# pixray/pixray

Hardware: AMD Instinct MI355X
Metric: optimisation iters/sec, VQGAN 256^2 + ViT-B/32 + 64 cutouts (higher is better)
Workload: dtype fp16

## Files before the change

### include/prx.h

```cpp
#ifndef PRX_H_
#define PRX_H_
#include <stddef.h>
#include <stdint.h>

#ifdef __cplusplus
extern "C" {
#endif

#define PRX_ABI_VERSION 3

typedef void* prx_stream_t;

const char* prx_last_error(void);
int prx_abi_version(void);
int prx_device_info(int* cu_count, char* arch_name, int arch_name_len);


#define PRX_ACT_NONE 0
#define PRX_ACT_QUICKGELU 1
#define PRX_ACT_MUL_DQUICKGELU 2
#define PRX_ACT_RELU 3
#define PRX_ACT_MUL_RELUMASK 4
#define PRX_ACT_RELUMASK_POST 5
#define PRX_ACT_GELU 6
// ... 106 lines not shown
int prx_k_image_head_bwd_im2col(const float* x, int ldc, const float* gimg, void* col, int ldk, int C, int H, int W, int h16,
                                const float* gscale, prx_stream_t s);
int prx_k_grad_scale(const float* g, size_t n, float* part, int nparts, int target_log2, float* scale2, prx_stream_t s);
int prx_k_grad_scale_multi(const float* const* gs, const size_t* ns, int count, float* part, int nparts_each, int target_log2,
                           float* scale2, prx_stream_t s);
int prx_k_scale_dev(float* x, size_t n, const float* scale, void* out16, int h16, prx_stream_t s);
int prx_k_f32_to_op16(const float* in, void* out16, size_t n, int h16, prx_stream_t s);
int prx_k_add_f32(const float* a, const float* b, float* out, size_t n, prx_stream_t s);

int prx_k_rn_pack_conv3x3(const float* w, void* Wf, void* Wd, int Cout, int Cin, int prec, prx_stream_t s);
int prx_k_stem1_fwd(const float* cut, const float* mm, const float* w, const float* b, void* out, int N, int S, int CO, int prec,
                    prx_stream_t s);
int prx_k_stem1_bwd(const void* g, const float* w, float* dY, int N, int S, int CO, const float* oscale_dev, int prec, prx_stream_t s);
int prx_k_avgpool2_fwd(const void* x, void* out, int N, int H, int W, int C, int prec, prx_stream_t s);
int prx_k_avgpool2_bwd(const float* g, const void* mask, float* dx_f32, void* dx_op, int N, int H, int W, int C, int prec,
                       prx_stream_t s);
int prx_k_relu_mask(float* g, const void* out, void* g_op, size_t n, int prec, prx_stream_t s);
int prx_k_tokens_fwd(const float* x, const float* pos, void* t, int N, int P, int C, int prec, prx_stream_t s);
int prx_k_tokens_bwd(const float* dt, float* dx, int N, int P, int C, int prec, prx_stream_t s);
int prx_k_tok0_gather(const void* t, void* out, int N, int T, int C, int prec, prx_stream_t s);
int prx_k_tok0_scatter(const void* g0, void* dt, int N, int T, int C, int prec, prx_stream_t s);
int prx_k_cnx_pack_dw(const float* w, void* pack, int C, int prec, prx_stream_t s);
int prx_k_cnx_dwconv(const void* x, const void* pack, const float* bias, const float* add, void* out_op, float* out_f32, int N, int H,
                     int W, int C, int flip, int prec, prx_stream_t s);
int prx_k_cnx_space_to_depth(const void* in, void* out, int N, int H, int W, int C, int prec, prx_stream_t s);
int prx_k_cnx_depth_to_space(const void* in, void* out, int N, int H, int W, int C, int prec, prx_stream_t s);
int prx_k_cnx_avgpool_fwd(const void* x, float* out, int N, int HW, int C, int prec, prx_stream_t s);
int prx_k_cnx_avgpool_bwd(const float* g, float* dx_f32, void* dx_op, int N, int HW, int C, int prec, prx_stream_t s);
int prx_k_cnx_layernorm_fwd(const void* x, int x_f32, const float* gamma, const float* beta, void* out_op, float* out_f32, float* mean,
                            float* rstd, int rows, int C, float eps, int group, int prec, prx_stream_t s);
int prx_k_cnx_layernorm_bwd(const float* g, const void* x, int x_f32, const float* gamma, const float* mean, const float* rstd,
                            void* dx_op, float* dx_f32, int rows, int C, int group, int prec, prx_stream_t s);
int prx_k_minmax(const float* x, size_t n, float* part, int nparts, float* mm, prx_stream_t s);
int prx_k_patchify_fwd(const float* cut, const float* mm, void* A, int prec, int N, int S, int P, int T, float m0, float m1, float m2,
                       float s0, float s1, float s2, prx_stream_t s);
int prx_k_patchify_bwd_reduce(const float* cut, const float* mm, const float* dA, double* acc, int N, int S, int P, int T, float m0,
                              float m1, float m2, float s0, float s1, float s2, prx_stream_t s);
int prx_k_patchify_bwd_apply(const float* cut, const float* mm, const float* dA, const double* acc, float* gcut, int N, int S, int P,
                             int T, float m0, float m1, float m2, float s0, float s1, float s2, prx_stream_t s);
int prx_k_preproc_bwd_reduce(const float* cut, const float* mm, const float* dY, double* acc, int N, int S, prx_stream_t s);
int prx_k_preproc_bwd_apply(const float* cut, const float* mm, const float* dY, const double* acc, float* gcut, int N, int S,
                            prx_stream_t s);
int prx_k_pool_fwd(const float* img, float* pooled, int* argmax, const unsigned char* mask, int C, int H, int W, int S, prx_stream_t s);
int prx_k_pool_bwd(const float* g, const int* argmax, const unsigned char* mask, float* gimg, int C, int H, int W, int S, prx_stream_t s);
int prx_k_rescale_fwd(const float* pooled, float* base, int C, int S, int Hb, int Wb, prx_stream_t s);
int prx_k_rescale_bwd(const float* g_base, float* g_pooled, int C, int S, int Hb, int Wb, prx_stream_t s);
int prx_k_warp_a_fwd(const float* src, int Hs, int Ws, const double* desc, float* out, int n_cut, int Ha, int Wa, prx_stream_t s);
int prx_k_warp_a_bwd(const float* g, int Hs, int Ws, const double* desc, float* uv, float* gsrc_priv, float* gsrc, int n_cut, int Ha,
                     int Wa, int form, prx_stream_t s);
int prx_k_warp_b_fwd(const float* a, int Ha, int Wa, const double* desc, const float* noise, float* out, int n_cut, int S,
                     prx_stream_t s);
int prx_k_warp_b_bwd(const float* a, int Ha, int Wa, const double* desc, const float* g, float* grgb, float* uv, float* ga, int n_cut,
                     int S, float* maps_scratch, size_t maps_scratch_bytes, int form, prx_stream_t s);
int prx_k_vgg_pack(const float* w, void* Wf, void* Wd, int Cout, int Cin, int CiP, int prec, prx_stream_t s);
int prx_k_vgg_input(const float* x, void* out, int HW, int prec, prx_stream_t s);
int prx_k_vgg_input_grad(const float* d, float* gx, int HW, const float* unscale, prx_stream_t s);
int prx_k_vgg_maxpool(const void* x, void* out, void* arg, int H, int W, int C, int prec, prx_stream_t s);
int prx_k_vgg_combine(const float* above, const void* arg, const float* gcap, const void* act, void* gpre, int H, int W, int C,
                      const float* gscale, int prec, prx_stream_t s);
int prx_k_pack_transpose_op(const float* in, void* out, int R, int C, int prec, prx_stream_t s);
int prx_k_vit_add_cls_pos(float* x, const float* cls, const float* pos, int N, int T, int W, prx_stream_t s);
int prx_k_vit_embed_tokens(const float* x, const float* cls, const float* pos, void* out, int out16, int N, int T, int W,
                           prx_stream_t s);
int prx_k_vit_gelu_f32(const float* t, float* io, size_t n, int bwd, prx_stream_t s);
int prx_k_vit_scale_f32(float* x, size_t n, float scale, int blocks, prx_stream_t s);
int prx_k_text_embed(const int* tokens, const float* emb, const float* pos, float* x, int* eot, int n, int ctx, int W, int vocab,
                     prx_stream_t s);
int prx_k_gather_rows(const float* x, const int* eot, float* out, int n, int ctx, int W, prx_stream_t s);
int prx_k_l2norm_fwd(const float* e, float* out, int n, int D, prx_stream_t s);
int prx_k_l2norm_bwd(const float* e, const float* g, float* de, int n, int D, prx_stream_t s);
int prx_k_vqgan_pack_conv3x3(const float* w, void* Wf, void* Wd, int Cout, int Cin, int CoP, int prec, prx_stream_t s);
int prx_k_vqgan_enc_pack_conv3x3(const float* w, void* Wf, int Cout, int Cin, int CiP, prx_stream_t s);
int prx_k_colminmax(const float* w, float* mn, float* mx, int rows, int D, prx_stream_t s);


typedef struct prx_vqgan prx_vqgan;
typedef struct prx_vqgan_config {
    int ch;
    int ch_mult[8];
    int n_mult;
    int num_res_blocks;
    int attn_resolution;
    int resolution;
    int z_channels;
    int embed_dim;
    int n_embed;
    int out_ch;
    int latent_h, latent_w;
    int precision;
} prx_vqgan_config;
int prx_vqgan_create(prx_vqgan** out, const prx_vqgan_config* cfg, const float* const* weights, int n_weights,
                     prx_stream_t s);
void prx_vqgan_destroy(prx_vqgan* h);
int prx_vqgan_z_bounds(prx_vqgan* h, float* zmin, float* zmax, prx_stream_t s);
int prx_vqgan_synth(prx_vqgan* h, const float* z, float* img, int* indices, int quantize, prx_stream_t s);
int prx_vqgan_synth_backward(prx_vqgan* h, const float* g_img, float* dz, prx_stream_t s);
long long prx_vqgan_debug_stage(prx_vqgan* h, int stage, float* dst, long long max_floats, prx_stream_t stream);

typedef struct prx_vqgan_enc prx_vqgan_enc;
int prx_vqgan_enc_create(prx_vqgan_enc** out, const prx_vqgan_config* cfg, int in_channels, int H, int W,
                         const float* const* weights, int n_weights, prx_stream_t s);
void prx_vqgan_enc_destroy(prx_vqgan_enc* h);
int prx_vqgan_encode(prx_vqgan_enc* h, const float* img, float* z, float* z_pre, int* indices, prx_stream_t s);

typedef struct prx_vgg16 prx_vgg16;
int prx_vgg16_create(prx_vgg16** out, const float* const* weights, int n_weights, int max_h, int max_w, int precision,
// ... 299 lines not shown
```

### pixray_amd/csrc/cutouts.hip

```cpp
#include "cutouts.h"
#include <algorithm>
#include <stdlib.h>
#include <stdio.h>

namespace {

constexpr int DESC_WORDS = 36;
enum { D_M1 = 0, D_M2 = 9, D_MODE1 = 18, D_MODE2 = 19, D_FILL = 20, D_JIT = 21, D_SAT = 22, D_HUE = 23,
       D_SATFIRST = 24, D_NOISE = 25, D_GRID1 = 26, D_GRID2 = 27,
       D_WOX = 28, D_WOY = 29, D_WW = 30, D_WH = 31,
       D_SEED = 32 };
enum { GRID_MESH = 0, GRID_AFFINE = 1, GRID_AFFINE_AC = 2, GRID_MESH_AC = 3 };
enum { MODE_IDENT = 0, MODE_ZEROS = 1, MODE_BORDER = 2, MODE_REFLECT = 3, MODE_FILL = 4,
       MODE_REFLECT_AC = 5 };

inline int ew_grid(size_t total) { return (int)std::min<size_t>((total + 255) / 256, 16384); }

__device__ __forceinline__ int win_start(int i, int in, int out) { return (int)(((long long)i * in) / out); }
__device__ __forceinline__ int win_end(int i, int in, int out) { return (int)((((long long)(i + 1)) * in + out - 1) / out); }

__global__ __launch_bounds__(256) void pool_fwd_kernel(const float* __restrict__ img, float* __restrict__ pooled,
                                                       int* __restrict__ argmax, const unsigned char* __restrict__ mask,
                                                       int C, int H, int W, int S) {
    const int total = C * S * S;
    for (int idx = blockIdx.x * blockDim.x + threadIdx.x; idx < total; idx += gridDim.x * blockDim.x) {
        const int x = idx % S, y = (idx / S) % S, c = idx / (S * S);
        const int y0 = win_start(y, H, S), y1 = win_end(y, H, S);
        const int x0 = win_start(x, W, S), x1 = win_end(x, W, S);
        float sum = 0.f, mx = -INFINITY;
        int am = y0 * W + x0;
        for (int yy = y0; yy < y1; ++yy)
            for (int xx = x0; xx < x1; ++xx) {
                float v = img[((size_t)c * H + yy) * W + xx];
                sum += v;
                if (v > mx || v != v) { mx = v; am = yy * W + xx; }
            }
        pooled[idx] = (mask && mask[idx]) ? 0.f : 0.5f * (sum / (float)((y1 - y0) * (x1 - x0)) + mx);
        argmax[idx] = am;
    }
}

__global__ __launch_bounds__(256) void pool_bwd_kernel(const float* __restrict__ g, const int* __restrict__ argmax,
                                                       const unsigned char* __restrict__ mask, float* __restrict__ gimg, int C, int H,
                                                       int W, int S) {
    const int total = C * H * W;
    for (int idx = blockIdx.x * blockDim.x + threadIdx.x; idx < total; idx += gridDim.x * blockDim.x) {
        const int xx = idx % W, yy = (idx / W) % H, c = idx / (H * W);
        int ya = (int)(((long long)yy * S) / H), xa = (int)(((long long)xx * S) / W);
        while (ya > 0 && win_end(ya - 1, H, S) > yy) --ya;
        while (xa > 0 && win_end(xa - 1, W, S) > xx) --xa;
        float acc = 0.f;
        for (int y = ya; y < S && win_start(y, H, S) <= yy; ++y) {
            const int y0 = win_start(y, H, S), y1 = win_end(y, H, S);
            if (yy >= y1) continue;
// ... 479 lines not shown
            }
        }
    if (COOP) {
#pragma unroll
        for (int c = 0; c < 3; ++c)
#pragma unroll
            for (int o = 32; o > 0; o >>= 1) acc[c] += __shfl_xor(acc[c], o, 64);
    }
    return total;
}

__device__ __forceinline__ void gather_tile(const GatherStage& st, const StageMap& sm, TileStage& ts, int tx0, int ty0, int sx, int sy,
                                            bool live, float (&out)[3]) {
    if (threadIdx.x == 0) {
        int x0, x1, y0, y1;
        ts.w = 0; ts.h = 0; ts.x0 = 0; ts.y0 = 0;
        const float ua = fmaxf((float)tx0 - 1.f, sm.ulo), ub = fminf((float)(tx0 + TILE_W) + 1.f, sm.uhi);
        const float va = fmaxf((float)ty0 - 1.f, sm.vlo), vb = fminf((float)(ty0 + TILE_W) + 1.f, sm.vhi);
        if (ub > ua && vb > va && preimage_box(sm, ua, ub, va, vb, st.Wd, st.Hd, x0, x1, y0, y1) &&
            (x1 - x0 + 1) * (y1 - y0 + 1) <= STAGE_CAP) {
            ts.x0 = x0; ts.y0 = y0; ts.w = x1 - x0 + 1; ts.h = y1 - y0 + 1;
        }
    }
    __syncthreads();
    {
        const int cnt = ts.w * ts.h;
        const size_t plane = (size_t)st.Hd * st.Wd;
        for (int k = threadIdx.x; k < cnt; k += 256) {
            const size_t o = (size_t)(ts.y0 + k / ts.w) * st.Wd + (ts.x0 + k % ts.w);
            ts.uv[k] = st.uv[o];
            ts.g[0][k] = st.g[o]; ts.g[1][k] = st.g[plane + o]; ts.g[2][k] = st.g[2 * plane + o];
        }
    }
    __syncthreads();
    float acc[3] = {0.f, 0.f, 0.f};
    int work = 0;
    if (live) work = gather_pixel<false>(st, sm, ts, sx, sy, acc, HEAVY);
    unsigned long long heavy = __ballot(live && work > HEAVY);
    while (heavy) {
        const int src = __ffsll((long long)heavy) - 1;
        heavy &= heavy - 1;
        const int hx = __shfl(sx, src, 64), hy = __shfl(sy, src, 64);
        float a2[3] = {0.f, 0.f, 0.f};
        gather_pixel<true>(st, sm, ts, hx, hy, a2, 0);
        if ((int)(threadIdx.x & 63) == src) { acc[0] = a2[0]; acc[1] = a2[1]; acc[2] = a2[2]; }
    }
    out[0] = acc[0]; out[1] = acc[1]; out[2] = acc[2];
}

struct TileRects {
    float ua[MAXR * MAXR], ub[MAXR * MAXR], va[MAXR * MAXR], vb[MAXR * MAXR];
    int x0[MAXR * MAXR], y0[MAXR * MAXR], bw[MAXR * MAXR], cnt[MAXR * MAXR];
};
struct TileScatter {
    int nrect;
    TileRects rect;
    float acc[4][3][TILE_W * TILE_W];
};
struct WaveScatter {
    TileRects rect;
    float acc[3][TILE_W * TILE_W];
};

__device__ __forceinline__ void scatter_candidate(const GatherStage& st, float* __restrict__ a0, float* __restrict__ a1, float* __restrict__ a2,
                                                  int tx0, int ty0, float ua, float ub, float va, float vb, float2 q, float g0, float g1, float g2) {
    if (!(q.x >= ua && q.x < ub && q.y >= va && q.y < vb)) return;
    const Taps t = make_taps(q.x, q.y, st.Ws, st.Hs, st.mode);
    const int lx = t.x0 - tx0, ly = t.y0 - ty0;
    const bool cx0 = t.vx0 && lx >= 0 && lx < TILE_W, cx1 = t.vx1 && lx + 1 >= 0 && lx + 1 < TILE_W;
    const bool cy0 = t.vy0 && ly >= 0 && ly < TILE_W, cy1 = t.vy1 && ly + 1 >= 0 && ly + 1 < TILE_W;
    if (!((cx0 || cx1) && (cy0 || cy1))) return;
    const float e = 1.f - t.wx, s_ = 1.f - t.wy;
    const float w00 = s_ * e, w01 = s_ * t.wx, w10 = t.wy * e, w11 = t.wy * t.wx;
    const int p00 = ly * TILE_W + lx;
    if (cx0 && cy0) { atomicAdd(&a0[p00], g0 * w00); atomicAdd(&a1[p00], g1 * w00); atomicAdd(&a2[p00], g2 * w00); }
    if (cx1 && cy0) { atomicAdd(&a0[p00 + 1], g0 * w01); atomicAdd(&a1[p00 + 1], g1 * w01); atomicAdd(&a2[p00 + 1], g2 * w01); }
    if (cx0 && cy1) { atomicAdd(&a0[p00 + TILE_W], g0 * w10); atomicAdd(&a1[p00 + TILE_W], g1 * w10); atomicAdd(&a2[p00 + TILE_W], g2 * w10); }
    if (cx1 && cy1) { atomicAdd(&a0[p00 + TILE_W + 1], g0 * w11); atomicAdd(&a1[p00 + TILE_W + 1], g1 * w11); atomicAdd(&a2[p00 + TILE_W + 1], g2 * w11); }
}

template <int STRIDE>
__device__ __forceinline__ void scatter_rect(const GatherStage& st, const TileRects& tr, int r, int tid, float* __restrict__ a0,
                                             float* __restrict__ a1, float* __restrict__ a2, int tx0, int ty0) {
    constexpr int U = 4;
    const size_t plane = (size_t)st.Hd * st.Wd;
    const float ua = tr.ua[r], ub = tr.ub[r], va = tr.va[r], vb = tr.vb[r];
    const int bx0 = tr.x0[r], by0 = tr.y0[r], bw = tr.bw[r], cnt = tr.cnt[r];
    const float ibw = 1.f / (float)bw;
    for (int k0 = tid; k0 < cnt; k0 += STRIDE * U) {
        float2 q[U]; float g0[U], g1[U], g2[U];
#pragma unroll
        for (int j = 0; j < U; ++j) {
            const int k = k0 + STRIDE * j;
            q[j] = make_float2(-INFINITY, -INFINITY);
            g0[j] = g1[j] = g2[j] = 0.f;
            if (k < cnt) {
                int ky = (int)((float)k * ibw);
                int kx = k - ky * bw;
                if (kx < 0) { --ky; kx += bw; } else if (kx >= bw) { ++ky; kx -= bw; }
                const size_t o = (size_t)(by0 + ky) * st.Wd + (bx0 + kx);
                q[j] = st.uv[o];
                g0[j] = st.g[o]; g1[j] = st.g[plane + o]; g2[j] = st.g[2 * plane + o];
            }
        }
#pragma unroll
        for (int j = 0; j < U; ++j) scatter_candidate(st, a0, a1, a2, tx0, ty0, ua, ub, va, vb, q[j], g0[j], g1[j], g2[j]);
    }
}

__device__ __forceinline__ void scatter_tile(const GatherStage& st, const StageMap& sm, TileScatter& ts, int tx0, int ty0, float (&out)[3]) {
    const int tid = threadIdx.x, wave = tid >> 6;
    if (tid == 0) {
        int n = 0;
        const int sx0 = max(tx0, 0), sx1 = min(tx0 + TILE_W - 1, st.Ws - 1);
        const int sy0 = max(ty0, 0), sy1 = min(ty0 + TILE_W - 1, st.Hs - 1);
        if (sx0 <= sx1 && sy0 <= sy1) {
            float xa[MAXR], xb[MAXR], ya[MAXR], yb[MAXR];
            const int nx = tile_intervals(st.mode, sx0, sx1, st.Ws, sm.ulo, sm.uhi, xa, xb);
            const int ny = tile_intervals(st.mode, sy0, sy1, st.Hs, sm.vlo, sm.vhi, ya, yb);
            for (int j = 0; j < ny; ++j)
                for (int i = 0; i < nx; ++i) {
                    int x0, x1, y0, y1;
                    if (!preimage_box(sm, xa[i], xb[i], ya[j], yb[j], st.Wd, st.Hd, x0, x1, y0, y1)) continue;
                    ts.rect.ua[n] = xa[i]; ts.rect.ub[n] = xb[i]; ts.rect.va[n] = ya[j]; ts.rect.vb[n] = yb[j];
                    ts.rect.x0[n] = x0; ts.rect.y0[n] = y0; ts.rect.bw[n] = x1 - x0 + 1; ts.rect.cnt[n] = (x1 - x0 + 1) * (y1 - y0 + 1);
                    ++n;
                }
        }
        ts.nrect = n;
    }
#pragma unroll
    for (int c = 0; c < 3; ++c)
#pragma unroll
        for (int w = 0; w < 4; ++w) ts.acc[w][c][tid] = 0.f;
    __syncthreads();
    const int nrect = ts.nrect;
    for (int r = 0; r < nrect; ++r) scatter_rect<256>(st, ts.rect, r, tid, ts.acc[wave][0], ts.acc[wave][1], ts.acc[wave][2], tx0, ty0);
    __syncthreads();
#pragma unroll
    for (int c = 0; c < 3; ++c) out[c] = ((ts.acc[0][c][tid] + ts.acc[1][c][tid]) + ts.acc[2][c][tid]) + ts.acc[3][c][tid];
}

__device__ __forceinline__ void scatter_tile_wave(const GatherStage& st, const StageMap& sm, WaveScatter& ts, int tx0, int ty0, float (&out)[4][3]) {
    const int lane = threadIdx.x & 63;
#pragma unroll
    for (int c = 0; c < 3; ++c)
#pragma unroll
        for (int j = 0; j < 4; ++j) ts.acc[c][lane + 64 * j] = 0.f;
    if (lane < MAXR * MAXR) {
        int cnt = 0;
        const int sx0 = max(tx0, 0), sx1 = min(tx0 + TILE_W - 1, st.Ws - 1);
        const int sy0 = max(ty0, 0), sy1 = min(ty0 + TILE_W - 1, st.Hs - 1);
        if (sx0 <= sx1 && sy0 <= sy1) {
            float xa[MAXR], xb[MAXR], ya[MAXR], yb[MAXR];
            const int nx = tile_intervals(st.mode, sx0, sx1, st.Ws, sm.ulo, sm.uhi, xa, xb);
            const int ny = tile_intervals(st.mode, sy0, sy1, st.Hs, sm.vlo, sm.vhi, ya, yb);
            const int i = lane % MAXR, j = lane / MAXR;
            if (i < nx && j < ny) {
                const float ua = i == 0 ? xa[0] : (i == 1 ? xa[1] : xa[2]), ub = i == 0 ? xb[0] : (i == 1 ? xb[1] : xb[2]);
                const float va = j == 0 ? ya[0] : (j == 1 ? ya[1] : ya[2]), vb = j == 0 ? yb[0] : (j == 1 ? yb[1] : yb[2]);
                int x0, x1, y0, y1;
                if (preimage_box(sm, ua, ub, va, vb, st.Wd, st.Hd, x0, x1, y0, y1)) {
                    ts.rect.ua[lane] = ua; ts.rect.ub[lane] = ub; ts.rect.va[lane] = va; ts.rect.vb[lane] = vb;
                    ts.rect.x0[lane] = x0; ts.rect.y0[lane] = y0; ts.rect.bw[lane] = x1 - x0 + 1;
                    cnt = (x1 - x0 + 1) * (y1 - y0 + 1);
                }
            }
        }
        ts.rect.cnt[lane] = cnt;
    }
    __builtin_amdgcn_s_waitcnt(0xc07f);
    __builtin_amdgcn_wave_barrier();
    for (int r = 0; r < MAXR * MAXR; ++r) {
        if (ts.rect.cnt[r] == 0) continue;
        scatter_rect<64>(st, ts.rect, r, lane, ts.acc[0], ts.acc[1], ts.acc[2], tx0, ty0);
    }
    __builtin_amdgcn_s_waitcnt(0xc07f);
    __builtin_amdgcn_wave_barrier();
#pragma unroll
    for (int j = 0; j < 4; ++j)
#pragma unroll
        for (int c = 0; c < 3; ++c) out[j][c] = ts.acc[c][lane + 64 * j];
}

__device__ __forceinline__ void write_stage_map(StageMap* __restrict__ maps, int n, const StageWords& w, int Wd, int Hd, int Ws, int Hs) {
    if (maps == nullptr || blockIdx.x != 0 || threadIdx.x != 0) return;
    StageMap sm{};
    if (w.mode != MODE_IDENT) build_stage_map(sm, w.m, w.gtype, Wd, Hd, Ws, Hs);
    maps[n] = sm;
}

__global__ __launch_bounds__(256) void uv_kernel(const double* __restrict__ desc, float2* __restrict__ uv, StageMap* __restrict__ maps,
                                                 int Wd, int Hd, int Ws, int Hs) {
// ... 107 lines not shown
    const StageWords w = stage_words(d, 2);
    const SrcWin q = src_window(d);
    write_stage_map(maps, n, w, S, S, q.ww, q.wh);
    const bool jit = d[D_JIT] != 0.0;
    if (w.mode == MODE_IDENT && !jit) return;
    const unsigned plane = (unsigned)S * (unsigned)S, stride = gridDim.x * blockDim.x;
    float2* uvn = uv + (size_t)n * plane;
    if (!jit) {
        for (unsigned pix = blockIdx.x * blockDim.x + threadIdx.x; pix < plane; pix += stride) {
            int x, y;
            pixel_xy(pix, (unsigned)S, x, y);
            float u, v;
            project(w.m, w.gtype, x, y, S, S, q.ww, q.wh, u, v);
            uvn[pix] = make_float2(u, v);
        }
        return;
    }
    const bool sat_first = d[D_SATFIRST] != 0.0;
    const float sat = (float)d[D_SAT], hue = (float)d[D_HUE];
    const size_t aplane = (size_t)Ha * Wa;
    const float* an = a + (size_t)n * 3 * aplane + (size_t)q.oy * Wa + q.ox;
    const float* gn = g + (size_t)n * 3 * plane;
    float* grn = grgb + (size_t)n * 3 * plane;
    for (unsigned pix = blockIdx.x * blockDim.x + threadIdx.x; pix < plane; pix += stride) {
        int x, y;
        pixel_xy(pix, (unsigned)S, x, y);
        Taps t = ident_taps(x, y);
        if (w.mode != MODE_IDENT) {
            float u, v;
            project(w.m, w.gtype, x, y, S, S, q.ww, q.wh, u, v);
            uvn[pix] = make_float2(u, v);
            t = make_taps(u, v, q.ww, q.wh, w.mode);
        }
        const float fillc = fill_term(t, w.fillv);
        Dual<3> rgb[3];
        float gin[3];
#pragma unroll
        for (int c = 0; c < 3; ++c) {
            rgb[c] = cst<3>(sample_plane(an + c * aplane, Wa, t) + fillc);
            rgb[c].d[c] = 1.f;
            gin[c] = gn[(size_t)c * plane + pix];
        }
        jitter_d<3>(rgb, sat, hue, sat_first);
#pragma unroll
        for (int i = 0; i < 3; ++i)
            grn[(size_t)i * plane + pix] = gin[0] * rgb[0].d[i] + gin[1] * rgb[1].d[i] + gin[2] * rgb[2].d[i];
    }
}

template <int FORM, int STAGE>
__global__ __launch_bounds__(FORM == 1 ? 64 : 256) void warp_bwd_kernel(const double* __restrict__ desc, const float* __restrict__ g,
                                                                        const float* __restrict__ grgb, const float2* __restrict__ uv,
                                                                        const StageMap* __restrict__ maps, float* __restrict__ out,
                                                                        int Wd, int Hd, int Wo, int Ho) {
    constexpr int NT = FORM == 1 ? 64 : 256;
    constexpr int PPT = TILE_W * TILE_W / NT;
    const int n = blockIdx.y;
    const double* d = desc + (size_t)n * DESC_WORDS;
    const int mode = (int)d[STAGE == 1 ? D_MODE1 : D_MODE2];
    const int ox = STAGE == 1 ? 0 : (int)d[D_WOX], oy = STAGE == 1 ? 0 : (int)d[D_WOY];
    const int ww = STAGE == 1 ? Wo : (int)d[D_WW], wh = STAGE == 1 ? Ho : (int)d[D_WH];
    const auto in_window = [&](int sx, int sy) { return STAGE == 1 || (sx >= 0 && sx < ww && sy >= 0 && sy < wh); };
    const size_t plane = (size_t)Hd * Wd, oplane = (size_t)Ho * Wo;
    const float* gi = (STAGE == 2 && d[D_JIT] != 0.0 ? grgb : g) + (size_t)n * 3 * plane;
    float* go = out + (size_t)n * 3 * oplane;
    const int tiles = (Wo + TILE_W - 1) / TILE_W;
    const int ax0 = (blockIdx.x % tiles) * TILE_W, ay0 = (blockIdx.x / tiles) * TILE_W;
    float o[PPT][3];
    if (mode == MODE_IDENT) {
#pragma unroll
        for (int j = 0; j < PPT; ++j) {
            const int p = threadIdx.x + NT * j, ax = ax0 + (p & 15), ay = ay0 + (p >> 4), sx = ax - ox, sy = ay - oy;
            const bool live = ax < Wo && ay < Ho && in_window(sx, sy) && sx < Wd && sy < Hd;
#pragma unroll
            for (int c = 0; c < 3; ++c) o[j][c] = live ? gi[(size_t)c * plane + (size_t)sy * Wd + sx] : 0.f;
        }
    } else {
        const GatherStage st{mode, Wd, Hd, ww, wh, gi, uv + (size_t)n * plane};
        const int tx0 = ax0 - ox, ty0 = ay0 - oy;
        if constexpr (FORM == 2) {
            __shared__ StageMap sm;
            __shared__ TileStage ts;
            if (threadIdx.x == 0) build_stage_map(sm, d + (STAGE == 1 ? D_M1 : D_M2), (int)d[STAGE == 1 ? D_GRID1 : D_GRID2], Wd, Hd, ww, wh);
            __syncthreads();
            const int ax = ax0 + (threadIdx.x & 15), ay = ay0 + (threadIdx.x >> 4), sx = ax - ox, sy = ay - oy;
            gather_tile(st, sm, ts, tx0, ty0, sx, sy, ax < Wo && ay < Ho && in_window(sx, sy), o[0]);
        } else if constexpr (FORM == 0) {
            __shared__ TileScatter ts;
            const StageMap sm = maps[n];
            scatter_tile(st, sm, ts, tx0, ty0, o[0]);
        } else {
            __shared__ WaveScatter ts;
            const StageMap sm = maps[n];
            scatter_tile_wave(st, sm, ts, tx0, ty0, o);
        }
    }
#pragma unroll
    for (int j = 0; j < PPT; ++j) {
        const int p = threadIdx.x + NT * j, ax = ax0 + (p & 15), ay = ay0 + (p >> 4);
        if (!(ax < Wo && ay < Ho)) continue;
        const bool live = in_window(ax - ox, ay - oy);
#pragma unroll
        for (int c = 0; c < 3; ++c) go[(size_t)c * oplane + (size_t)ay * Wo + ax] = live ? o[j][c] : 0.f;
    }
}

__device__ __forceinline__ void resize_taps(int o, int in, int outn, int& i0, int& i1, float& w1) {
    float src = ((float)o + 0.5f) * ((float)in / (float)outn) - 0.5f;
    if (src < 0.f) src = 0.f;
    i0 = (int)src;
    i1 = i0 + (i0 < in - 1 ? 1 : 0);
    w1 = src - (float)i0;
}
__global__ __launch_bounds__(256) void rescale_fwd_kernel(const float* __restrict__ p, float* __restrict__ out, int C, int S, int Hb, int Wb) {
    const size_t total = (size_t)C * Hb * Wb;
    for (size_t idx = (size_t)blockIdx.x * blockDim.x + threadIdx.x; idx < total; idx += (size_t)gridDim.x * blockDim.x) {
        const int x = (int)(idx % Wb), y = (int)((idx / Wb) % Hb), c = (int)(idx / ((size_t)Hb * Wb));
        int x0, x1, y0, y1; float wx, wy;
        resize_taps(x, S, Wb, x0, x1, wx); resize_taps(y, S, Hb, y0, y1, wy);
        const float* q = p + (size_t)c * S * S;
        out[idx] = (1.f - wy) * ((1.f - wx) * q[y0 * S + x0] + wx * q[y0 * S + x1]) + wy * ((1.f - wx) * q[y1 * S + x0] + wx * q[y1 * S + x1]);
    }
}
__device__ __forceinline__ void rescale_run(int s, int in, int outn, int& o0, int& o1) {
    const float sc = (float)outn / (float)in;
    o0 = max((int)floorf(((float)s - 1.f + 0.5f) * sc - 0.5f) - 1, 0);
    o1 = min((int)ceilf(((float)s + 1.f + 0.5f) * sc - 0.5f) + 1, outn - 1);
}
__global__ __launch_bounds__(256) void rescale_bwd_kernel(const float* __restrict__ g, float* __restrict__ gp, int C, int S, int Hb, int Wb) {
    const size_t total = (size_t)C * S * S;
    for (size_t idx = (size_t)blockIdx.x * blockDim.x + threadIdx.x; idx < total; idx += (size_t)gridDim.x * blockDim.x) {
        const int sx = (int)(idx % S), sy = (int)((idx / S) % S), c = (int)(idx / ((size_t)S * S));
        int xa, xb, ya, yb;
        rescale_run(sx, S, Wb, xa, xb); rescale_run(sy, S, Hb, ya, yb);
        const float* q = g + (size_t)c * Hb * Wb;
        float acc = 0.f;
        for (int y = ya; y <= yb; ++y) {
            int y0, y1; float wy;
            resize_taps(y, S, Hb, y0, y1, wy);
            const float cy = (y0 == sy ? (1.f - wy) : 0.f) + (y1 == sy ? wy : 0.f);
            if (cy == 0.f) continue;
            for (int x = xa; x <= xb; ++x) {
                int x0, x1; float wx;
// ... 173 lines not shown
    if (threadIdx.x < 4)
        atomicAdd(&acc[threadIdx.x], (red[0][threadIdx.x] + red[1][threadIdx.x]) + (red[2][threadIdx.x] + red[3][threadIdx.x]));
}

template <bool VEC>
__global__ __launch_bounds__(256) void patchify_bwd_apply_kernel(const float* __restrict__ cut,
                                                                 const float* __restrict__ mm,
                                                                 const float* __restrict__ dA,
                                                                 const double* __restrict__ acc, float* __restrict__ gcut,
                                                                 int N, int S, int P, int T, int K, PatchNorm nm) {
    constexpr int W = VEC ? 4 : 1;
    const int G = S / P;
    const float mn = mm[0], mx = mm[1];
    const float range = mx - mn;
    const bool live = range != 0.f;
    const float inv = live ? 1.f / range : 1.f;
    const float gmin = live ? (float)((acc[1] - acc[0]) * inv / fmax(acc[2], 1.0)) : 0.f;
    const float gmax = live ? (float)(-acc[1] * inv / fmax(acc[3], 1.0)) : 0.f;
    const unsigned per_plane = (unsigned)S * (unsigned)S / W, stride = gridDim.x * blockDim.x;
    for (unsigned pl = blockIdx.y; pl < (unsigned)N * 3u; pl += gridDim.y) {
        const int n = (int)(pl / 3u), c = (int)(pl - 3u * n);
        const float sd = nm.std[c];
        for (unsigned e = blockIdx.x * blockDim.x + threadIdx.x; e < per_plane; e += stride) {
            const RenormQuad r = renorm_decode<VEC>(e, pl, n, c, S, P, G, T, K);
            float xv[W], ga[W], go[W];
            if constexpr (VEC) {
                const float4 x4 = *reinterpret_cast<const float4*>(cut + r.idx), g4 = *reinterpret_cast<const float4*>(dA + r.ia);
                xv[0] = x4.x; xv[1] = x4.y; xv[2] = x4.z; xv[3] = x4.w;
                ga[0] = g4.x; ga[1] = g4.y; ga[2] = g4.z; ga[3] = g4.w;
            } else {
                xv[0] = cut[r.idx]; ga[0] = dA[r.ia];
            }
#pragma unroll
            for (int j = 0; j < W; ++j) {
                const float gy = ga[j] / sd;
                float g = gy * inv;
                if (xv[j] == mn) g += gmin;
                if (xv[j] == mx) g += gmax;
                go[j] = g;
            }
            if constexpr (VEC) *reinterpret_cast<float4*>(gcut + r.idx) = make_float4(go[0], go[1], go[2], go[3]);
            else gcut[r.idx] = go[0];
        }
    }
}

}

static int cutout_bwd_form(int form) {
    static const int env = [] { const char* e = getenv("PRX_CUTOUT_BWD"); return !e ? 0 : e[0] == 'g' ? 2 : e[0] == 'w' ? 1 : 0; }();
    return form < 0 ? env : form;
}

template <int STAGE>
static int launch_warp_bwd(int form, const double* desc, const float* g, const float* grgb, const float2* uv, StageMap* maps, float* out,
                           int n_cut, int Wd, int Hd, int Wo, int Ho, hipStream_t s) {
    const dim3 grid(((Wo + TILE_W - 1) / TILE_W) * ((Ho + TILE_W - 1) / TILE_W), n_cut);
    if (form == 2)
        hipLaunchKernelGGL((warp_bwd_kernel<2, STAGE>), grid, dim3(256), 0, s, desc, g, grgb, uv, nullptr, out, Wd, Hd, Wo, Ho);
    else if (form == 0)
        hipLaunchKernelGGL((warp_bwd_kernel<0, STAGE>), grid, dim3(256), 0, s, desc, g, grgb, uv, maps, out, Wd, Hd, Wo, Ho);
    else
        hipLaunchKernelGGL((warp_bwd_kernel<1, STAGE>), grid, dim3(64), 0, s, desc, g, grgb, uv, maps, out, Wd, Hd, Wo, Ho);
    PRX_LAUNCH_CHECK();
    return 0;
}

int prx_pool_fwd(const float* img, float* pooled, int* argmax, const unsigned char* mask, int C, int H, int W, int S, hipStream_t s) {
    hipLaunchKernelGGL(pool_fwd_kernel, dim3(ew_grid((size_t)C * S * S)), dim3(256), 0, s, img, pooled, argmax, mask, C, H, W, S);
    PRX_LAUNCH_CHECK();
    return 0;
}
int prx_pool_bwd(const float* g, const int* argmax, const unsigned char* mask, float* gimg, int C, int H, int W, int S, hipStream_t s) {
    hipLaunchKernelGGL(pool_bwd_kernel, dim3(ew_grid((size_t)C * H * W)), dim3(256), 0, s, g, argmax, mask, gimg, C, H, W, S);
    PRX_LAUNCH_CHECK();
    return 0;
}
#define PRX_REQUIRE_PLANE32(what, n_cut, H, W)                                                                                   \
    do {                                                                                                                         \
        PRX_REQUIRE((size_t)(H) * (size_t)(W) < ((size_t)1 << 31), what ": a plane of %dx%d exceeds the 32-bit index range", H, W); \
        PRX_REQUIRE((n_cut) <= 65535, what ": %d cutouts exceed the 65535 rows of a launch grid", n_cut);                        \
    } while (0)
static inline dim3 plane_grid(size_t plane, int n_cut, int max_blocks) {
    return dim3(std::min(ew_grid(plane), max_blocks), n_cut);
}

int prx_warp_a_fwd(const float* src, int Hs, int Ws, const double* desc, float* out, int n_cut, int Ha, int Wa, hipStream_t s) {
    PRX_REQUIRE_PLANE32("warp_a_fwd", n_cut, Ha, Wa);
    PRX_REQUIRE_PLANE32("warp_a_fwd (source)", n_cut, Hs, Ws);
    hipLaunchKernelGGL(warp_a_fwd_kernel, plane_grid((size_t)Ha * Wa, n_cut, 1024), dim3(256), 0, s, src, Hs, Ws, desc, out,
                       n_cut, Ha, Wa);
    PRX_LAUNCH_CHECK();
    return 0;
}
int prx_warp_a_bwd(const float* g, int Hs, int Ws, const double* desc, float* uv, float* gsrc_priv, float* gsrc, int n_cut, int Ha,
                   int Wa, hipStream_t s, int form) {
    PRX_REQUIRE(form >= -1 && form <= 2, "warp_a_bwd: form is not one of -1, 0, 1, 2");
    form = cutout_bwd_form(form);
    if (form != 2)
        PRX_REQUIRE((size_t)n_cut * sizeof(StageMap) <= (size_t)3 * Hs * Ws * sizeof(float), "warp_a_bwd: too many cutouts for the stage-map scratch");
    PRX_REQUIRE_PLANE32("warp_a_bwd", n_cut, Ha, Wa);
    hipLaunchKernelGGL(uv_kernel, plane_grid((size_t)Ha * Wa, n_cut, 64), dim3(256), 0, s, desc, (float2*)uv,
                       form != 2 ? (StageMap*)gsrc : nullptr, Wa, Ha, Ws, Hs);
    PRX_LAUNCH_CHECK();
    if (int rc = launch_warp_bwd<1>(form, desc, g, nullptr, (const float2*)uv, (StageMap*)gsrc, gsrc_priv, n_cut, Wa, Ha, Ws, Hs, s)) return rc;
    hipLaunchKernelGGL(reduce_planes_kernel, dim3((unsigned)std::min<size_t>(((size_t)3 * Hs * Ws + 63) / 64, 65536)), dim3(64), 0, s,
                       gsrc_priv, gsrc, n_cut, (size_t)3 * Hs * Ws);
    PRX_LAUNCH_CHECK();
    return 0;
}
int prx_warp_b_fwd(const float* a, int Ha, int Wa, const double* desc, const float* noise, float* out, int n_cut, int S,
                   hipStream_t s) {
    PRX_REQUIRE_PLANE32("warp_b_fwd", n_cut, S, S);
    hipLaunchKernelGGL(warp_b_fwd_kernel, plane_grid((size_t)S * S, n_cut, 1024), dim3(256), 0, s, a, Ha, Wa, desc, noise, out,
                       n_cut, S);
    PRX_LAUNCH_CHECK();
// ... 95 lines not shown
```

Before: 167.3.

## Add separable fast path for axis-aligned affine cutout warp backward

For affine warp stages with negligible off-diagonal terms and zero or fill padding, the FORM 0 backward kernel now handles each tile with a separable scheme. It computes per-axis source coordinates and per-output-pixel tap ranges, optionally stages the gradient block in shared memory, and sums weighted contributions directly. This replaces the general rect-based scatter with four accumulators. The default order (2) reproduces the scatter summation order so results stay matching. It adds shared memory (a union over the accumulator array), an extra check pass and a fallback path when the coordinates are not truly separable.

```diff
diff --git a/include/prx.h b/include/prx.h
--- a/include/prx.h
+++ b/include/prx.h
@@ -182,6 +182,7 @@
                      prx_stream_t s);
 int prx_k_warp_b_bwd(const float* a, int Ha, int Wa, const double* desc, const float* g, float* grgb, float* uv, float* ga, int n_cut,
                      int S, float* maps_scratch, size_t maps_scratch_bytes, int form, prx_stream_t s);
+int prx_cutout_bwd_separable(int on);
 int prx_k_vgg_pack(const float* w, void* Wf, void* Wd, int Cout, int Cin, int CiP, int prec, prx_stream_t s);
 int prx_k_vgg_input(const float* x, void* out, int HW, int prec, prx_stream_t s);
 int prx_k_vgg_input_grad(const float* d, float* gx, int HW, const float* unscale, prx_stream_t s);
diff --git a/pixray_amd/csrc/cutouts.hip b/pixray_amd/csrc/cutouts.hip
--- a/pixray_amd/csrc/cutouts.hip
+++ b/pixray_amd/csrc/cutouts.hip
@@ -1,5 +1,6 @@
 #include "cutouts.h"
 #include <algorithm>
+#include <atomic>
 #include <stdlib.h>
 #include <stdio.h>
 
@@ -585,10 +586,29 @@
     float ua[MAXR * MAXR], ub[MAXR * MAXR], va[MAXR * MAXR], vb[MAXR * MAXR];
     int x0[MAXR * MAXR], y0[MAXR * MAXR], bw[MAXR * MAXR], cnt[MAXR * MAXR];
 };
+constexpr int SEP_CAP = 80;
+constexpr int SEP_G_CAP = 1600;
+constexpr double SEP_OFFDIAG = 0x1p-40;
+__device__ __forceinline__ bool separable_stage(const double* m, int gtype, int mode) {
+    if (gtype != GRID_AFFINE && gtype != GRID_AFFINE_AC) return false;
+    if (mode != MODE_ZEROS && mode != MODE_FILL) return false;
+    return fabs(m[1]) <= SEP_OFFDIAG && fabs(m[3]) <= SEP_OFFDIAG;
+}
+struct TileSeparable {
+    float u[SEP_CAP], v[SEP_CAP];
+    int xlo[TILE_W], xhi[TILE_W];
+    int ylo[TILE_W], yhi[TILE_W];
+    int differs[4];
+};
+
 struct TileScatter {
     int nrect;
     TileRects rect;
-    float acc[4][3][TILE_W * TILE_W];
+    union {
+        float acc[4][3][TILE_W * TILE_W];
+        float g[3][SEP_G_CAP];
+    };
+    TileSeparable sep;
 };
 struct WaveScatter {
     TileRects rect;
@@ -672,6 +692,130 @@
     __syncthreads();
 #pragma unroll
     for (int c = 0; c < 3; ++c) out[c] = ((ts.acc[0][c][tid] + ts.acc[1][c][tid]) + ts.acc[2][c][tid]) + ts.acc[3][c][tid];
+}
+
+template <bool STAGED>
+__device__ __forceinline__ void separable_sum(const GatherStage& st, const TileScatter& ts, int x0, int y0, int bw, int tx0, int ty0, float (&acc)[3]) {
+    const int kx = threadIdx.x & 15, ky = threadIdx.x >> 4, sx = tx0 + kx, sy = ty0 + ky;
+    const int xl = ts.sep.xlo[kx], xh = ts.sep.xhi[kx], yl = ts.sep.ylo[ky], yh = ts.sep.yhi[ky];
+    const size_t plane = (size_t)st.Hd * st.Wd;
+    for (int j = yl; j <= yh; ++j) {
+        const float wy = tap_weight(ts.sep.v[j], sy);
+        if (wy == 0.f) continue;
+        const float* gr = st.g + (size_t)(y0 + j) * st.Wd + x0;
+        for (int i = xl; i <= xh; ++i) {
+            const float w = wy * tap_weight(ts.sep.u[i], sx);
+            float g0, g1, g2;
+            if (STAGED) { const int li = j * bw + i; g0 = ts.g[0][li]; g1 = ts.g[1][li]; g2 = ts.g[2][li]; }
+            else { g0 = gr[i]; g1 = gr[plane + i]; g2 = gr[2 * plane + i]; }
+            if (w == 0.f) continue;
+            acc[0] += g0 * w; acc[1] += g1 * w; acc[2] += g2 * w;
+        }
+    }
+}
+template <bool STAGED>
+__device__ __forceinline__ void separable_sum_scatter_order(const GatherStage& st, const TileScatter& ts, int x0, int y0, int bw, int tx0, int ty0,
+                                                            float (&acc)[3]) {
+    const int kx = threadIdx.x & 15, ky = threadIdx.x >> 4, sx = tx0 + kx, sy = ty0 + ky;
+    const int xl = ts.sep.xlo[kx], xh = ts.sep.xhi[kx], yl = ts.sep.ylo[ky], yh = ts.sep.yhi[ky];
+    if (xl > xh || yl > yh) return;
+    const size_t plane = (size_t)st.Hd * st.Wd;
+    const int bmin = (yl * bw + xl) >> 6, bmax = (yh * bw + xh) >> 6;
+#pragma unroll
+    for (int wave = 0; wave < 4; ++wave) {
+        float p[3] = {0.f, 0.f, 0.f};
+        for (int b = bmin + ((wave - bmin) & 3); b <= bmax; b += 4) {
+            const int klo = b << 6, khi = klo + 63;
+            for (int kind = 0; kind < 4; ++kind)
+                for (int j = yl; j <= yh; ++j) {
+                    const int ilo = max(xl, klo - j * bw), ihi = min(xh, khi - j * bw);
+                    if (ilo > ihi) continue;
+                    const float v = ts.sep.v[j];
+                    if ((v - (float)sy < 0.f) != ((kind >> 1) != 0)) continue;
+                    const float wy = tap_weight(v, sy);
+                    if (wy == 0.f) continue;
+                    const float* gr = st.g + (size_t)(y0 + j) * st.Wd + x0;
+                    for (int i = ilo; i <= ihi; ++i) {
+                        const float u = ts.sep.u[i];
+                        if ((u - (float)sx < 0.f) != ((kind & 1) != 0)) continue;
+                        const float w = wy * tap_weight(u, sx);
+                        if (w == 0.f) continue;
+                        float g0, g1, g2;
+                        if (STAGED) { const int li = j * bw + i; g0 = ts.g[0][li]; g1 = ts.g[1][li]; g2 = ts.g[2][li]; }
+                        else { g0 = gr[i]; g1 = gr[plane + i]; g2 = gr[2 * plane + i]; }
+                        p[0] += g0 * w; p[1] += g1 * w; p[2] += g2 * w;
+                    }
+                }
+        }
+#pragma unroll
+        for (int c = 0; c < 3; ++c) acc[c] = wave == 0 ? p[c] : acc[c] + p[c];
+    }
+}
+__device__ __forceinline__ bool separable_tile(const GatherStage& st, const StageMap& sm, TileScatter& ts, int tx0, int ty0, bool live, int order,
+                                               float (&out)[3]) {
+    const int tid = threadIdx.x;
+    int x0 = 0, x1 = -1, y0 = 0, y1 = -1;
+    bool any = false;
+    const int sx0 = max(tx0, 0), sx1 = min(tx0 + TILE_W - 1, st.Ws - 1);
+    const int sy0 = max(ty0, 0), sy1 = min(ty0 + TILE_W - 1, st.Hs - 1);
+    if (sx0 <= sx1 && sy0 <= sy1) {
+        float xa[MAXR], xb[MAXR], ya[MAXR], yb[MAXR];
+        const int nx = tile_intervals(st.mode, sx0, sx1, st.Ws, sm.ulo, sm.uhi, xa, xb);
+        const int ny = tile_intervals(st.mode, sy0, sy1, st.Hs, sm.vlo, sm.vhi, ya, yb);
+        if (nx && ny) any = preimage_box(sm, xa[0], xb[0], ya[0], yb[0], st.Wd, st.Hd, x0, x1, y0, y1);
+    }
+    const int bw = any ? x1 - x0 + 1 : 0, bh = any ? y1 - y0 + 1 : 0;
+    if (bw > SEP_CAP || bh > SEP_CAP) return false;
+    const bool staged = bw * bh <= SEP_G_CAP;
+    bool differs = false;
+    if (tid < 128) {
+        if (tid < bw) {
+            const float a = st.uv[(size_t)y0 * st.Wd + x0 + tid].x, b = st.uv[(size_t)y1 * st.Wd + x0 + tid].x;
+            ts.sep.u[tid] = a;
+            differs = __float_as_uint(a) != __float_as_uint(b);
+        }
+    } else if (tid - 128 < bh) {
+        const size_t row = (size_t)(y0 + tid - 128) * st.Wd;
+        const float a = st.uv[row + x0].y, b = st.uv[row + x1].y;
+        ts.sep.v[tid - 128] = a;
+        differs = __float_as_uint(a) != __float_as_uint(b);
+    }
+    const bool wave_differs = __ballot(differs) != 0;
+    if ((tid & 63) == 0) ts.sep.differs[tid >> 6] = wave_differs;
+    if (staged) {
+        const size_t plane = (size_t)st.Hd * st.Wd;
+        for (int ly = tid >> 5; ly < bh; ly += 8)
+            for (int lx = tid & 31; lx < bw; lx += 32) {
+                const size_t o = (size_t)(y0 + ly) * st.Wd + x0 + lx;
+                const int li = ly * bw + lx;
+                ts.g[0][li] = st.g[o]; ts.g[1][li] = st.g[plane + o]; ts.g[2][li] = st.g[2 * plane + o];
+            }
+    }
+    __syncthreads();
+    if (ts.sep.differs[0] | ts.sep.differs[1] | ts.sep.differs[2] | ts.sep.differs[3]) return false;
+    if (tid < 2 * TILE_W) {
+        const bool rows = tid >= TILE_W;
+        const int k = tid & (TILE_W - 1), s = (rows ? ty0 : tx0) + k, cnt = rows ? bh : bw;
+        const float* tab = rows ? ts.sep.v : ts.sep.u;
+        int lo = cnt, hi = -1;
+        for (int i = 0; i < cnt; ++i)
+            if (tap_weight(tab[i], s) != 0.f) { lo = min(lo, i); hi = i; }
+        (rows ? ts.sep.ylo : ts.sep.xlo)[k] = lo;
+        (rows ? ts.sep.yhi : ts.sep.xhi)[k] = hi;
+    }
+    __syncthreads();
+    float acc[3] = {0.f, 0.f, 0.f};
+    if (live) {
+        if (order == 2) {
+            if (staged) separable_sum_scatter_order<true>(st, ts, x0, y0, bw, tx0, ty0, acc);
+            else separable_sum_scatter_order<false>(st, ts, x0, y0, bw, tx0, ty0, acc);
+        } else {
+            if (staged) separable_sum<true>(st, ts, x0, y0, bw, tx0, ty0, acc);
+            else separable_sum<false>(st, ts, x0, y0, bw, tx0, ty0, acc);
+        }
+    }
+    out[0] = acc[0]; out[1] = acc[1]; out[2] = acc[2];
+    return true;
 }
 
 __device__ __forceinline__ void scatter_tile_wave(const GatherStage& st, const StageMap& sm, WaveScatter& ts, int tx0, int ty0, float (&out)[4][3]) {
@@ -885,7 +1029,7 @@
 __global__ __launch_bounds__(FORM == 1 ? 64 : 256) void warp_bwd_kernel(const double* __restrict__ desc, const float* __restrict__ g,
                                                                         const float* __restrict__ grgb, const float2* __restrict__ uv,
                                                                         const StageMap* __restrict__ maps, float* __restrict__ out,
-                                                                        int Wd, int Hd, int Wo, int Ho) {
+                                                                        int Wd, int Hd, int Wo, int Ho, int sep) {
     constexpr int NT = FORM == 1 ? 64 : 256;
     constexpr int PPT = TILE_W * TILE_W / NT;
     const int n = blockIdx.y;
@@ -921,7 +1065,12 @@
         } else if constexpr (FORM == 0) {
             __shared__ TileScatter ts;
             const StageMap sm = maps[n];
-            scatter_tile(st, sm, ts, tx0, ty0, o[0]);
+            bool done = false;
+            if (sep && separable_stage(d + (STAGE == 1 ? D_M1 : D_M2), (int)d[STAGE == 1 ? D_GRID1 : D_GRID2], mode)) {
+                const int ax = ax0 + (threadIdx.x & 15), ay = ay0 + (threadIdx.x >> 4);
+                done = separable_tile(st, sm, ts, tx0, ty0, ax < Wo && ay < Ho && in_window(ax - ox, ay - oy), sep, o[0]);
+            }
+            if (!done) scatter_tile(st, sm, ts, tx0, ty0, o[0]);
         } else {
             __shared__ WaveScatter ts;
             const StageMap sm = maps[n];
@@ -1201,16 +1350,25 @@
     return form < 0 ? env : form;
 }
 
+static std::atomic<int> g_cutout_bwd_sep{[] {
+    const char* e = getenv("PRX_CUTOUT_BWD_SEP");
+    return !e ? 2 : e[0] == '0' ? 0 : e[0] == '1' ? 1 : 2;
+}()};
+extern "C" int prx_cutout_bwd_separable(int on) {
+    return on < 0 ? g_cutout_bwd_sep.load(std::memory_order_relaxed) : g_cutout_bwd_sep.exchange(on > 2 ? 2 : on);
+}
+
 template <int STAGE>
 static int launch_warp_bwd(int form, const double* desc, const float* g, const float* grgb, const float2* uv, StageMap* maps, float* out,
                            int n_cut, int Wd, int Hd, int Wo, int Ho, hipStream_t s) {
     const dim3 grid(((Wo + TILE_W - 1) / TILE_W) * ((Ho + TILE_W - 1) / TILE_W), n_cut);
     if (form == 2)
-        hipLaunchKernelGGL((warp_bwd_kernel<2, STAGE>), grid, dim3(256), 0, s, desc, g, grgb, uv, nullptr, out, Wd, Hd, Wo, Ho);
+        hipLaunchKernelGGL((warp_bwd_kernel<2, STAGE>), grid, dim3(256), 0, s, desc, g, grgb, uv, nullptr, out, Wd, Hd, Wo, Ho, 0);
     else if (form == 0)
-        hipLaunchKernelGGL((warp_bwd_kernel<0, STAGE>), grid, dim3(256), 0, s, desc, g, grgb, uv, maps, out, Wd, Hd, Wo, Ho);
+        hipLaunchKernelGGL((warp_bwd_kernel<0, STAGE>), grid, dim3(256), 0, s, desc, g, grgb, uv, maps, out, Wd, Hd, Wo, Ho,
+                           g_cutout_bwd_sep.load(std::memory_order_relaxed));
     else
-        hipLaunchKernelGGL((warp_bwd_kernel<1, STAGE>), grid, dim3(64), 0, s, desc, g, grgb, uv, maps, out, Wd, Hd, Wo, Ho);
+        hipLaunchKernelGGL((warp_bwd_kernel<1, STAGE>), grid, dim3(64), 0, s, desc, g, grgb, uv, maps, out, Wd, Hd, Wo, Ho, 0);
     PRX_LAUNCH_CHECK();
     return 0;
 }
```

Measured after the change: 169.6, median of 6. 1.4% higher.
